# Illumina/manta

Hardware: AMD Instinct MI355X
Metric: candidate SV loci assembled+aligned per second (whole node) (higher is better)
Workload: dtype int32

## Files before the change

### manta_amd/csrc/api_internal.hpp

```cpp
#pragma once
#include "../../include/manta_amd.h"

#include <algorithm>
#include <atomic>
#include <functional>
#include <condition_variable>
#include <chrono>
#include <cstdio>
#include <cstdlib>
#include <cstring>
#include <memory>
#include <mutex>
#include <optional>
#include <string>
#include <thread>
#include <vector>

#include "align_kernels.hpp"
#include "align_jump_pair.hpp"
#include "assemble_kernels.hpp"
#include "asm_lds.hpp"
#include "small_asm.hpp"
#include "pipeline_kernels.hpp"
#include "split_kernels.hpp"
// ... 866 lines not shown
    P.bits_cap       = devBitsCap;
    P.bits_used      = reinterpret_cast<unsigned long long*>(dCnt + 2);
    P.phase_cycles   = reinterpret_cast<unsigned long long*>(dCnt + 4);
    P.growth_size    = dGrowth;
    P.growth_buckets = dGrowth + ctx->growthSize.size();
    P.n_growth       = uint32_t(ctx->growthSize.size());
    P.flags          = std::getenv("MANTA_AMD_SERIAL_WALK") ? ASM_FLAG_SERIAL_WALK : 0u;
    P.locus_min_wl   = dMinWl;
    P.locus_max_wl   = dMaxWl;
    P.locus_ids      = dOrder;
    P.pl_codes       = dPlCodes;
    P.pl_nmask       = dPlMask;
    P.pl_read_len    = dPlLen;
    P.pl_code_off    = dPlCodeOff;
    P.pl_mask_off    = dPlMaskOff;
    chunks.fill(P);
    P.reserved2          = 0;
    P.small_min_seed_reads = smallMinSeedReads;
    P.small_max_iterations = smallMaxIterations;
    P.punt_ids             = nullptr;
    P.punt_count           = nullptr;
    P.n_loci_dev           = nullptr;
    P.lds_bytes            = ASM_LDS_BYTES;
    P.stop_before          = 0;
    lastParams             = P;
    nRerun                 = 0;
    if (smallMode) {
      rt::launch(small_assemble_kernel, grid, 0, P);
      return;
    }
    int g = grid;
    if (chunks.active() && g >= ctx->cuCount * 16) g = rt::roundGrid(g - ctx->cuCount);
    P.lds_bytes = ASM_LDS_BYTES;
    if (useFast) {
      using namespace manta_dev;
      const uint32_t nGen = uint32_t(genIds.size());
      rt::h2d(reinterpret_cast<uint32_t*>(dCnt + 14), &nGen, sizeof(uint32_t));
      uint64_t* dLg = bLgCnt.as<uint64_t>(16);
      rt::dzero(dLg, sizeof(uint64_t) * 16);
      LgArgs A;
      A.P            = P;
      A.P.n_loci     = uint32_t(fastIds.size());
      A.P.punt_ids   = dPunt;
      A.P.punt_count = reinterpret_cast<uint32_t*>(dCnt + 14);
      A.G.arena        = bLgArena.as<uint8_t>(lgArenaCap + 64);
      A.G.arena_cap    = lgArenaCap;
      A.G.arena_used   = reinterpret_cast<unsigned long long*>(dLg);
      A.G.slab_off     = bLgOff.as<uint64_t>(nLoci);
      A.G.class_ids    = bLgClassIds.as<uint32_t>(uint64_t(LG_CLASSES) * std::max<size_t>(1, fastIds.size()));
      A.G.class_count  = reinterpret_cast<uint32_t*>(dLg + 1);
      A.G.class_stride = uint32_t(fastIds.size());
      for (unsigned c = 0; c < LG_CLASSES; ++c) A.G.class_bytes[c] = classBytes[c];
      A.G.cls        = 0;
      A.G.flags      = (std::getenv("MANTA_AMD_LG_NO_PROOF") ? LG_FLAG_NO_PROOF : 0u) | (std::getenv("MANTA_AMD_LG_NO_RESCUE") ? LG_FLAG_NO_RESCUE : 0u);
      A.G.stats      = reinterpret_cast<uint32_t*>(dLg + 8);
      int maxGrid = 1;
      for (unsigned c = 0; c < LG_CLASSES; ++c) maxGrid = std::max(maxGrid, gridContig[c]);
      A.G.cws        = bCws.as<uint8_t>(cwsStride * uint64_t(maxGrid));
      A.G.cws_stride = cwsStride;
      A.G.cost_bins = nullptr;
      if (contigPool && !fastIds.empty()) {
        A.G.cost_bins = bLgBins.as<uint32_t>(CK_BIN_IDS + uint64_t(CK_BINS) * fastIds.size());
        rt::dzero(A.G.cost_bins, sizeof(uint32_t) * CK_BIN_IDS);
      }
      A.G.round = A.G.last_round = 0;
      A.G.iter        = nullptr;
      A.G.parena      = nullptr;
      A.G.parena_cap  = 0;
      A.G.parena_used = nullptr;
      A.G.next_ids = A.G.next_count = A.G.cyc_ids = A.G.cyc_count = nullptr;
      A.G.rws        = nullptr;
      A.G.rws_stride = 0;
      A.G.gws        = nullptr;
      A.G.rprof      = nullptr;
      A.G.sched      = sched;
      int gf = gridFast;
      if (chunks.active() && gf >= ctx->cuCount * 2) gf -= ChunkStream::streamFreeSlots(ctx->cuCount);
      if (!fastIds.empty()) {
        uint32_t firstWl = opt.min_word_length;
        if (!locusMinWl.empty()) {
          firstWl = 0;
          for (const uint32_t l : fastIds) firstWl = std::max(firstWl, locusMinWl[l]);
        }
        if (firstWl <= 32)
          rt::launchWG(graph_kernel<2>, gf, int(LG_WAVES), LG_BUDGET, A);
        else if (firstWl <= 64)
          rt::launchWG(graph_kernel<4>, gf, int(LG_WAVES), LG_BUDGET, A);
        else
          rt::launchWG(graph_kernel<8>, gf, int(LG_WAVES), LG_BUDGET, A);
      }
      bool smallContigsLaunched = false;
      auto launchSmallContigs   = [&] {
        if (smallContigsLaunched) return;
        smallContigsLaunched = true;
        if (sched && schedWaits) rt::curStreamWaits(*schedWaits);
        for (unsigned c = 0; c < LG_CLASSES && !fastIds.empty(); ++c) {
          if (!classBytes[c]) continue;
          A.G.cls       = c;
          A.P.counter   = reinterpret_cast<uint32_t*>(dLg + 3) + c;
          A.P.lds_bytes = classBytes[c];
          if (c == 0 && contigPool)
            rt::launchWG(contig_pool_kernel, gridContig[c] / int(CK_POOL_WAVES), int(CK_POOL_WAVES), CK_POOL_BYTES, A);
          else
            rt::launchSingle(contig_kernel, gridContig[c], classBytes[c], A);
        }
      };
      firstRoundHookRan = false;
// ... 237 lines not shown
    seqCopied  = std::min<uint64_t>(cnt[1], devSeqCap);
    bitsCopied = std::min<uint64_t>(cnt[2], devBitsCap);
    hSeq       = pSeq.as<uint8_t>(seqCopied + 1);
    hBits      = pBits.as<uint64_t>(bitsCopied + 1);
    rt::d2hAsync(hCnt, dCnt, sizeof(uint64_t) * 16);
    rt::d2hAsync(hLoci, dLoci, sizeof(AsmLocusOut) * nLoci);
    rt::d2hAsync(hCont, dCont, sizeof(AsmContigOut) * uint64_t(nLoci) * opt.max_assembly_count);
    rt::d2hAsync(hSeq, dSeq, seqCopied);
    rt::d2hAsync(hBits, dBits, sizeof(uint64_t) * bitsCopied);
    done.record();
    earlyStaged = true;
  }
  void finishEarly()
  {
    seqUsedDev  = seqCopied;
    bitsUsedDev = bitsCopied;
    seqLast     = seqUsedDev;
    bitsLast    = bitsUsedDev;
    stagedTotals();
  }
  template <typename F0>
  void stageEnqueueRest(F0 firstCopies)
  {
    firstCopies();
    stageQueued = true;
  }
  void stagedTotals()
  {
    nContigsOut = pseudoBytesOut = pseudoCountOut = 0;
    for (uint32_t l = 0; l < nLoci; ++l) {
      const AsmLocusOut& h(hLoci[l]);
      if (h.status != ASM_OK) continue;
      nContigsOut += h.n_contigs;
      pseudoCountOut += h.n_pseudo;
      for (uint32_t q = 0; q < h.n_pseudo; ++q) pseudoBytesOut += hBits[h.pseudo_len_off + q];
    }
    staged = true;
    ldsFallbacks = useFast ? uint32_t(hCnt[14] & 0xffffffffu) - uint32_t(genIds.size()) : 0u;
    if (std::getenv("MANTA_AMD_DEBUG") && useFast) {
      uint32_t st[2] = {0, 0}, stBig[10] = {0, 0, 0, 0, 0, 0, 0, 0, 0, 0}, clsBig[2] = {0, 0};
      rt::d2h(st, bLgCnt.as<uint64_t>(16) + 8, sizeof(st));
      rt::d2h(stBig, bLgCnt.as<uint64_t>(16) + 11, sizeof(stBig));
      rt::d2h(clsBig, bLgCnt.as<uint64_t>(16) + 5, sizeof(clsBig));
      std::fprintf(stderr, "manta_amd: LDS assembler pipeline: %zu + %zu (big class) loci, %u handed to the general kernel (+ %zu outside its envelope); %u + %u graphs came "
                           "with a proof of acyclicity, %u + %u reads re-anchored; big class: %u / %u loci in its two contig LDS classes\n", fastIds.size(), bigIds.size(),
                   ldsFallbacks, genIds.size(), st[0], stBig[0], st[1], stBig[1], clsBig[0], clsBig[1]);
      if (contigPool && !fastIds.empty()) {
        uint32_t bins[manta_dev::CK_BIN_IDS];
        rt::d2h(bins, bLgBins.as<uint32_t>(manta_dev::CK_BIN_IDS + uint64_t(manta_dev::CK_BINS) * fastIds.size()), sizeof(bins));
        const uint32_t* ps = bins + manta_dev::CK_BIN_STAT;
        std::fprintf(stderr, "manta_amd: contig_pool_kernel: %u shares taken, %.2f loci resident per CU on average at a take, %u takes waited for room (%u polls); "
                             "loci by cost bin (largest first):", ps[0], ps[0] ? double(ps[1]) / ps[0] : 0.0, ps[2], ps[3]);
        for (unsigned b = 0; b < manta_dev::CK_BINS; ++b) std::fprintf(stderr, " %u", bins[b]);
        std::fprintf(stderr, "\n");
      }
      if (!bigIds.empty())
        std::fprintf(stderr, "manta_amd: big class, %u word-length rounds; handed back: %u envelope, %u table / set pool, %u words / side tables / class, %u slab arena, %u by "
                             "repeat_big_kernel, %u by contig_big_kernel, %u pseudo arena, %u out of rounds\n", bigRounds, stBig[2], stBig[3], stBig[4], stBig[5], stBig[6],
                     stBig[7], stBig[8], stBig[9]);
      if (bigRounds) {
        unsigned long long rp[8] = {0, 0, 0, 0, 0, 0, 0, 0}, tot = 0;
        uint32_t           perRound[8 * manta_dev::LGL_MAX_ROUNDS];
        uint32_t*          rc = bLgRounds.as<uint32_t>(8 * (manta_dev::LGL_MAX_ROUNDS + 1) + 32);
        rt::d2h(rp, rc + 8 * (manta_dev::LGL_MAX_ROUNDS + 1), sizeof(rp));
        rt::d2h(perRound, rc, sizeof(perRound));
        for (int i = 0; i < 7; ++i) tot += rp[i];
        std::fprintf(stderr, "manta_amd: repeat_big_kernel clocks: renumbering %.1f%% component scan %.1f%% hash+insertion %.1f%% order1 %.1f%% order2 %.1f%% search in the reference's order %.1f%% rest %.1f%% (%.0f k clocks per graph without a proof, first three rounds)\n",
                     tot ? 100.0 * rp[0] / tot : 0, tot ? 100.0 * rp[1] / tot : 0, tot ? 100.0 * rp[2] / tot : 0, tot ? 100.0 * rp[3] / tot : 0, tot ? 100.0 * rp[4] / tot : 0,
                     tot ? 100.0 * rp[5] / tot : 0, tot ? 100.0 * rp[6] / tot : 0, perRound[5] ? double(tot) / 1e3 / double(std::max<uint32_t>(1, perRound[5] + perRound[8 + 5] + perRound[16 + 5])) : 0.0);
        std::fprintf(stderr, "manta_amd: rounds (graphs without a proof / loci sent on):");
        for (uint32_t r = 0; r < bigRounds; ++r) std::fprintf(stderr, " %u/%u", perRound[8 * r + 5], perRound[8 * r + 7]);
        std::fprintf(stderr, "\n");
      }
    }
    if (std::getenv("MANTA_AMD_PROFILE")) {
      static const char* namesGeneral[8] = {"pack", "table", "links", "cycle-check", "exact", "seed", "walk", "select+emit"};
#ifdef MANTA_LG_PROFILE_GRAPH
      static const char* namesLds[8]     = {"pack", "table", "links", "counts+radix", "ties+ids", "slab+sets+init", "preds+sibs", "spec+write"};
#else
      static const char* namesLds[8]     = {"pack", "table", "sort+records", "cycle-check", "slab write/read", "seed+replay", "walk", "select+emit"};
#endif
      const char* const* names = useFast ? namesLds : namesGeneral;
      uint64_t           tot = 0;
      for (int i = 0; i < 8; ++i) tot += hCnt[4 + i];
      std::fprintf(stderr, "manta_amd %s phase share (shader clocks summed over %u loci; graph_kernel: clocks of one wave of the workgroup):", useFast ? "graph_kernel + contig_kernel" : "assemble_kernel", nLoci);
      for (int i = 0; i < 8; ++i) std::fprintf(stderr, " %s=%.1f%%", names[i], tot ? 100.0 * double(hCnt[4 + i]) / double(tot) : 0.0);
      std::fprintf(stderr, " | avg clocks/locus=%.0f\n", double(tot) / nLoci);
    }
  }
  void stageOut()
  {
    stageEnqueue([] {});
    rt::sync();
    stageFinish([](bool&) {});
  }

  struct SparseContigs {
    const AsmStage* st;
    const AsmContigOut& operator()(uint32_t l, uint32_t c) const { return st->hCont[uint64_t(l) * st->opt.max_assembly_count + c]; }
  };
  void exactSizes(uint64_t& nContigs, uint64_t& seqBytes, uint64_t& bitsWords) const { exactSizes(SparseContigs{this}, nContigs, seqBytes, bitsWords); }
  template <typename ContigAt>
  void exactSizes(ContigAt contigAt, uint64_t& nContigs, uint64_t& seqBytes, uint64_t& bitsWords) const
  {
    nContigs = nContigsOut;
    seqBytes = pseudoBytesOut;
    bitsWords = pseudoCountOut;
// ... 797 lines not shown
```

### manta_amd/csrc/asm_contig.hpp

```cpp
#pragma once
#ifdef MANTA_WAVE_EMU
#include <set>
#endif
#include "asm_lds.hpp"

namespace manta_dev {

#ifndef MANTA_CK_FAST_CAP
#define MANTA_CK_FAST_CAP 3
#endif
static const unsigned CK_FAST_CAP = MANTA_CK_FAST_CAP;
static const unsigned CK_MAX_EXT = 1020;

struct CkWsLayout {
  uint64_t lane_seq, lane_bits, lane_meta, lane_log, total;
};
static const unsigned CK_SEQ_WORDS = CK_MAX_EXT / 16 + 2;
static const unsigned CK_LOG_QW    = (CK_MAX_EXT + 4) / 4;
WV_HD CkWsLayout ckWorkspaceLayout(const unsigned setw = 2)
{
  CkWsLayout L;
  uint64_t   o = 0;
  L.lane_seq  = asmPut(o, 64ull * 2 * 4 * CK_SEQ_WORDS);
  L.lane_bits = asmPut(o, 64ull * 2 * setw * 8);
  L.lane_meta = asmPut(o, 64ull * 8 * 4);
  L.lane_log  = asmPut(o, 64ull * 8 * CK_LOG_QW);
  L.total     = (o + 255) & ~uint64_t(255);
  return L;
}

enum { CK_DONE = 0, CK_PUNT = 1, CK_NEXT = 2 };

template <class C>
struct LdsContig {
  typedef LgRec<C>  R;
  typedef FSetT<C>  Set;
  typedef CkMap<C>  M;
  static const unsigned SW  = C::SETW;
  static const unsigned IDB = C::ID_BITS;
  static const unsigned IDM = (1u << C::ID_BITS) - 1u;
  static const unsigned UPL = C::UNUSED_DW / 64;
  const AsmParams& P;
  const LgParams&  G;
  char*            lds;
  const uint8_t*   slab;
  FRec8*           nodes;
  Set*             pool;
  uint8_t*         rd1;
  uint32_t*        unused_bits;
  uint16_t *       tent, *slotNode, *sib, *sovf, *povf;
  LgSlab           SL;
  uint8_t*         tbl;
  uint32_t*        lane_seq;
  uint64_t*        lane_bits;
  int32_t*         lane_meta;
  uint64_t*        lane_log;
  unsigned         lane, nNormal, W, k, nNodes, nFat, nEligible, nSpec, nSib, nSovf, nPovf, codeWords, nCand, maxLen, seqWords;
  bool             acyclic;
  bool             cyclic, anyRep;
  unsigned         nPseudo, nCore, visDw;
  uint32_t *       coreBits, *repBits, *vis;
  uint16_t*        corePrefix;
  unsigned         candSlotV;
  uint64_t         tMark;
  unsigned         shareBytes;

  WV_DEV LdsContig(const AsmParams& p, const LgParams& g, char* base, uint8_t* ws) : P(p), G(g), lds(base)
  {
    lane        = unsigned(wv::lane());
    unused_bits = reinterpret_cast<uint32_t*>(lds + M::UNUSED);
    tent        = reinterpret_cast<uint16_t*>(lds + M::TENT);
    slotNode    = reinterpret_cast<uint16_t*>(lds + M::SLOTND);
    tbl         = reinterpret_cast<uint8_t*>(lds + M::TBL);
    sib         = reinterpret_cast<uint16_t*>(lds + M::SIB);
    sovf        = reinterpret_cast<uint16_t*>(lds + M::SOVF);
    povf        = reinterpret_cast<uint16_t*>(lds + M::POVF);
    nodes       = reinterpret_cast<FRec8*>(lds + M::RECS);
    pool        = nullptr;
    rd1         = nullptr;
    const CkWsLayout L = ckWorkspaceLayout(SW);
    lane_seq  = reinterpret_cast<uint32_t*>(ws + L.lane_seq);
    lane_bits = reinterpret_cast<uint64_t*>(ws + L.lane_bits);
    lane_meta = reinterpret_cast<int32_t*>(ws + L.lane_meta);
    lane_log  = reinterpret_cast<uint64_t*>(ws + L.lane_log);
    maxLen    = p.max_contig_len;
    seqWords  = CK_SEQ_WORDS;
    candSlotV = 0;
    nCand     = 0;
    shareBytes = 0;
    cyclic = anyRep = false;
    nPseudo = nCore = visDw = 0;
    coreBits = repBits = vis = nullptr;
    corePrefix = nullptr;
  }

  WV_DEV void tick(const int phase)
  {
#if defined(MANTA_ASM_PROFILE) && !defined(MANTA_LG_PROFILE_GRAPH)
    const uint64_t now = wv::clock();
    if (P.phase_cycles && lane == 0) wv::atomic_add(&P.phase_cycles[phase], (unsigned long long)(now - tMark));
    tMark = now;
#else
    (void)phase;
#endif
  }

  WV_DEV bool isUnused(const unsigned nd) const { return (unused_bits[nd >> 5] >> (nd & 31)) & 1u; }
  WV_DEV char*    scratch() const { return lds + M::RECS + ((8 * nNodes + 15) & ~15u) + (C::BIG ? ((nNodes + 15) & ~15u) : 0u); }

  WV_DEV unsigned onlyRead(const unsigned nd, const FRec8 w) const { return C::BIG ? unsigned(rd1[nd]) : lg8Read(w); }
  WV_DEV Set supOf(const unsigned nd, const FRec8 w) const
  {
    Set s;
    if (nd < nFat) {
      s = pool[nd];
    } else {
      const unsigned ref = onlyRead(nd, w);
      for (unsigned q = 0; q < SW; ++q) s.w[q] = ((ref >> 6) == q) ? (uint64_t(1) << (ref & 63)) : 0;
    }
    return s;
  }
  WV_DEV uint64_t succOf(const unsigned nd, const FRec8 w) const { return R::links(w, nd, true, sovf, nSovf); }
  WV_DEV uint64_t predOf(const unsigned nd, const FRec8 w) const { return R::links(w, nd, false, povf, nPovf); }
  WV_DEV static unsigned popSet(const Set& a)
  {
    unsigned n = 0;
    for (unsigned q = 0; q < SW; ++q) n += unsigned(wv::popc(a.w[q]));
    return n;
  }
  WV_DEV static Set setAnd(const Set& a, const Set& b)
  {
    Set r;
    for (unsigned q = 0; q < SW; ++q) r.w[q] = a.w[q] & b.w[q];
    return r;
  }
  WV_DEV static Set setAndNot(const Set& a, const Set& b)
  {
    Set r;
    for (unsigned q = 0; q < SW; ++q) r.w[q] = a.w[q] & ~b.w[q];
    return r;
  }
  WV_DEV static void setOrIn(Set& a, const Set& b)
  {
    for (unsigned q = 0; q < SW; ++q) a.w[q] |= b.w[q];
  }
  WV_DEV static Set setZero()
  {
    Set r;
    for (unsigned q = 0; q < SW; ++q) r.w[q] = 0;
    return r;
  }
  WV_DEV static Set setSel(const bool c, const Set& a, const Set& b)
  {
    Set r;
    for (unsigned q = 0; q < SW; ++q) r.w[q] = c ? a.w[q] : b.w[q];
    return r;
  }

  WV_DEV bool load(const unsigned locus)
  {
    slab            = G.arena + G.slab_off[locus];
    const LgHdr* gh = reinterpret_cast<const LgHdr*>(slab);
    nNodes          = wv::first(gh->nNodes);
    nFat            = wv::first(gh->nFat);
    k               = wv::first(gh->k);
    nNormal         = wv::first(gh->nNormal);
    nEligible       = wv::first(gh->nEligible);
    nSpec           = wv::first(gh->nSpec);
    nSib            = wv::first(gh->nSib);
    nSovf           = wv::first(gh->nSovf);
    nPovf           = wv::first(gh->nPovf);
    codeWords       = wv::first(gh->codeWords);
    W               = wv::first(gh->W);
    acyclic         = wv::first(gh->acyclic) != 0;
    cyclic          = C::BIG && wv::first(gh->cyclic) != 0;
    nPseudo         = C::BIG ? wv::first(gh->nPseudo) : 0u;
    nCore           = cyclic ? wv::first(gh->nCore) : 0u;
    if (wv::first(gh->need) > P.lds_bytes || nNodes > C::MAX_NODES) return false;
    SL               = lgSlabOf<C>(nNodes, nFat, codeWords);
    const FRec8* gRec = reinterpret_cast<const FRec8*>(slab + SL.recs);
    for (unsigned i = lane; i < nNodes; i += 64) nodes[i] = gRec[i];
    if (C::BIG) {
      rd1                 = reinterpret_cast<uint8_t*>(lds + M::RECS + ((8 * nNodes + 15) & ~15u));
      const uint32_t* g4  = reinterpret_cast<const uint32_t*>(slab + SL.rd1);
      uint32_t*       l4  = reinterpret_cast<uint32_t*>(rd1);
      for (unsigned i = lane; i < (nNodes + 3) / 4; i += 64) l4[i] = g4[i];
    }
    const uint16_t* gt = reinterpret_cast<const uint16_t*>(slab + SL.sib);
    for (unsigned i = lane; i < 4 * (LG_SIB_CAP + 2 * C::OVF_CAP); i += 64) sib[i] = gt[i];
    for (unsigned u = 0; u < UPL; ++u) {
      const unsigned d = UPL * lane + u, lo = 32 * d;
      unused_bits[d]   = (nEligible >= lo + 32) ? 0xffffffffu : ((nEligible > lo) ? ((1u << (nEligible - lo)) - 1u) : 0u);
    }
    if (cyclic) {
      char* x    = scratch() + 8 * SW * (nFat ? nFat : 1u);
      coreBits   = reinterpret_cast<uint32_t*>(x);
      corePrefix = reinterpret_cast<uint16_t*>(x + 4 * C::UNUSED_DW);
      repBits    = reinterpret_cast<uint32_t*>(x + 6 * C::UNUSED_DW);
      vis        = reinterpret_cast<uint32_t*>(x + 10 * C::UNUSED_DW);
      visDw      = (nCore + 31) / 32;
      const uint32_t* gf = reinterpret_cast<const uint32_t*>(slab + SL.flags);
      unsigned        c  = 0;
      uint32_t        cb[UPL];
      for (unsigned u = 0; u < UPL; ++u) {
        const unsigned d = UPL * lane + u;
        cb[u]            = gf[d];
        coreBits[d]      = cb[u];
        repBits[d]       = gf[C::UNUSED_DW + d];
        c += unsigned(wv::popc(cb[u]));
      }
      unsigned inc = c;
      for (int off = 1; off < 64; off <<= 1) {
        const unsigned o = wv::shfl(inc, int(lane) - off);
        if (int(lane) >= off) inc += o;
      }
      unsigned at = inc - c;
      for (unsigned u = 0; u < UPL; ++u) {
        corePrefix[UPL * lane + u] = uint16_t(at);
        at += unsigned(wv::popc(cb[u]));
      }
      wv::sync();
      for (unsigned u = 0; u < UPL; ++u) {
        uint32_t b32 = cb[u];
        while (b32) {
          const unsigned b = unsigned(wv::ctz(uint64_t(b32)));
          b32 &= b32 - 1;
          nodes[32 * (UPL * lane + u) + b] |= FRec8(1) << 63;
        }
      }
    }
    wv::sync();
    return true;
  }
  WV_DEV static bool coreFlag(const FRec8 w) { return C::BIG && (w >> 63) != 0; }
  WV_DEV unsigned    coreIndex(const unsigned nd) const
  {
    return unsigned(corePrefix[nd >> 5]) + unsigned(wv::popc(coreBits[nd >> 5] & ((1u << (nd & 31)) - 1u)));
  }
  WV_DEV const Set*      gPool() const { return reinterpret_cast<const Set*>(slab + SL.pool); }
  WV_DEV const uint16_t* gSpecList() const { return reinterpret_cast<const uint16_t*>(slab + SL.spec); }
  WV_DEV const uint16_t* gPb() const { return reinterpret_cast<const uint16_t*>(slab + SL.pb); }
  WV_DEV const uint32_t* gCodes() const { return reinterpret_cast<const uint32_t*>(slab + SL.codes); }

  WV_DEV void loadPool()
  {
    pool              = reinterpret_cast<Set*>(scratch());
    const Set* gp     = gPool();
    for (unsigned i = lane; i < nFat; i += 64) pool[i] = gp[i];
    if (nFat == 0 && lane == 0) pool[0] = setZero();
    wv::sync();
  }

  WV_DEV bool graphHasCycle()
  {
    const unsigned stDw = (nNodes + 3) / 4;
    uint32_t*      st    = reinterpret_cast<uint32_t*>(scratch());
    uint32_t*      qTail = st + stDw;
    uint16_t*      queue = reinterpret_cast<uint16_t*>(qTail + 4);
    if (lane == 0) *qTail = 0;
    for (unsigned w = lane; w < stDw; w += 64) st[w] = 0;
    wv::sync();
    for (unsigned nb = 0; nb < nNodes; nb += 64) {
      const unsigned nd = nb + lane;
      if (nd >= nNodes) continue;
      const FRec8    w  = nodes[nd];
      const uint64_t sl = succOf(nd, w), pl = predOf(nd, w);
      unsigned       id = 0, od = 0;
      for (unsigned c = 0; c < 4; ++c) {
        const unsigned s = R::linkId(sl, c), p = R::linkId(pl, c);
        if (s != ASM_NONE && s != nd) od++;
        if (p != ASM_NONE && p != nd) id++;
      }
      const bool     src = (id == 0 || od == 0);
      const unsigned v   = id | (od << 3) | (src ? 0x40u : 0u);
      wv::atomic_or(&st[nd >> 2], v << (8 * (nd & 3)));
      if (src) queue[wv::atomic_add(qTail, 1u)] = uint16_t(nd);
    }
    wv::sync();
    unsigned head = 0, removed = 0;
    while (true) {
      const unsigned tail = wv::first(wv::atomic_load(qTail));
      if (tail == head) break;
      removed += tail - head;
      for (unsigned i = head + lane; i < tail; i += 64) {
        const unsigned nd = queue[i];
        const FRec8    w  = nodes[nd];
        const uint64_t sl = succOf(nd, w), pl = predOf(nd, w);
        for (unsigned c = 0; c < 4; ++c) {
          const unsigned s = R::linkId(sl, c);
          if (s != ASM_NONE && s != nd) {
            const unsigned sh  = 8 * (s & 3);
            const unsigned old = wv::atomic_sub(&st[s >> 2], 1u << sh) >> sh;
            if ((old & 0x7u) == 1u && !(wv::atomic_or(&st[s >> 2], 0x40u << sh) & (0x40u << sh))) queue[wv::atomic_add(qTail, 1u)] = uint16_t(s);
          }
          const unsigned p = R::linkId(pl, c);
          if (p != ASM_NONE && p != nd) {
            const unsigned sh  = 8 * (p & 3);
            const unsigned old = wv::atomic_sub(&st[p >> 2], 8u << sh) >> sh;
            if ((old & 0x38u) == 8u && !(wv::atomic_or(&st[p >> 2], 0x40u << sh) & (0x40u << sh))) queue[wv::atomic_add(qTail, 1u)] = uint16_t(p);
          }
        }
      }
// ... 64 lines not shown
    unsigned ent[WIN], lab[WIN];
    for (unsigned h = 0; h < WIN; ++h) {
      const unsigned i = lane + 64 * h;
      ent[h]           = (i < nW) ? unsigned(tent[i]) : ASM_NONE;
      unsigned cur     = (i < nW) ? ent[h] : 0u;
      for (unsigned steps = 0; steps < 256 && i < nW; ++steps) {
        const FRec8    w  = nodes[cur];
        const unsigned f0 = R::succ(w, 0);
        if (f0 == 0 || R::succ(w, 1) != 0 || R::sOvf(w) || f0 - 1 == cur) break;
        const FRec8 wn = nodes[f0 - 1];
        if (R::pred(wn, 1) != 0 || R::pOvf(wn)) break;
        cur = f0 - 1;
      }
      lab[h] = (i < nW) ? cur : (ASM_NONE - 1u - i);
    }
    bool dup[WIN];
    for (unsigned h = 0; h < WIN; ++h) dup[h] = false;
    for (unsigned g = 0; g < WIN; ++g) {
      const unsigned gEnd = (nW > 64 * g) ? ((nW - 64 * g < 64) ? (nW - 64 * g) : 64u) : 0u;
      for (unsigned j = 0; j < gEnd; ++j) {
        const unsigned v = wv::readlane(lab[g], int(j));
        for (unsigned h = g; h < WIN; ++h)
          if (64 * g + j < lane + 64 * h && v == lab[h] && lane + 64 * h >= PLAIN) dup[h] = true;
      }
    }
    unsigned base = 0;
    uint64_t keepM[WIN];
    for (unsigned h = 0; h < WIN; ++h) keepM[h] = wv::ballot(ent[h] != ASM_NONE && !dup[h]);
#ifdef MANTA_WAVE_EMU
    if (emuWhy()) {
      for (unsigned h = 0; h < WIN; ++h)
        if (ent[h] != ASM_NONE) {
          dbg().looked.insert(ent[h]);
          if (dup[h]) dbg().dropped.insert(ent[h]);
        }
    }
#endif
    const uint64_t below = (uint64_t(1) << lane) - 1;
    wv::sync();
    for (unsigned h = 0; h < WIN; ++h) {
      if ((keepM[h] >> lane) & 1u) tent[base + unsigned(wv::popc(keepM[h] & below))] = uint16_t(ent[h]);
      base += unsigned(wv::popc(keepM[h]));
    }
    wv::sync();
    return (base < 64) ? base : 64u;
  }

  struct Cand {
    FRec8 w;
    Set   s;
  };

  WV_DEV FRec8    candRec(const unsigned f) const { return nodes[f ? f - 1 : 0]; }
  WV_DEV Set      candPool(const unsigned f) const { return pool[(f != 0 && f - 1 < nFat) ? f - 1 : 0u]; }
  WV_DEV unsigned candRd1(const unsigned f) const { return C::BIG ? unsigned(rd1[f ? f - 1 : 0]) : 0u; }
  WV_DEV Set      candSup(const unsigned f, const FRec8 w, const Set& p, const unsigned r1) const
  {
    const unsigned ref  = C::BIG ? r1 : lg8Read(w);
    const bool     fat  = f != 0 && f - 1 < nFat;
    const uint64_t useM = fat ? ~uint64_t(0) : 0;
    const uint64_t bit  = uint64_t((f != 0 && !fat) ? 1u : 0u) << (ref & 63);
    Set            s;
    if (SW == 2) {
      const uint64_t hiM = (ref & 64u) ? ~uint64_t(0) : 0;
      s.w[0]             = (p.w[0] & useM) | (bit & ~hiM);
      s.w[1]             = (p.w[1] & useM) | (bit & hiM);
    } else {
      for (unsigned q = 0; q < SW; ++q) s.w[q] = (p.w[q] & useM) | (((ref >> 6) == q) ? bit : 0);
    }
    return s;
  }
  WV_DEV Cand loadCand(const unsigned f) const
  {
    Cand           c;
    const Set      p  = candPool(f);
    const unsigned r1 = candRd1(f);
    c.w               = candRec(f);
    c.s               = candSup(f, c.w, p, r1);
    return c;
  }

  WV_DEV void walkSlots(const uint64_t walkMask)
  {
    const bool has = (walkMask >> lane) & 1u;
    LG_STAT(1, 1);
    LG_STAT(2, unsigned(wv::popc(walkMask)));
    const unsigned seed = has ? unsigned(slotNode[lane]) : 0u;
    uint64_t* const logBuf   = lane_log + lane;
    uint64_t        logAcc   = seed;
    uint32_t* const rightBuf = lane_seq + lane;
    uint32_t* const leftBuf  = lane_seq + 64 + lane;
    uint32_t       accR = 0, accL = 0;
    Set            S = setZero(), RJ = setZero();
    bool           active = has, rep = false, tooLong = false;
    unsigned       mode = 0, cur = seed, consOffset = 0, nLeft = 0, nRight = 0;
    int            consEnd = 0, consBegin = 0;
    FRec8          seedRec = 0;
    if (cyclic && has)
      for (unsigned w = 0; w < visDw; ++w) vis[w * 64 + lane] = 0;
    if (has) {
      seedRec = nodes[seed];
      S       = supOf(seed, seedRec);
      const bool repeatSeed = R::selfLoop(seedRec) || (cyclic && ((repBits[seed >> 5] >> (seed & 31)) & 1u));
      if (repeatSeed) {
        rep    = true;
        active = false;
      } else {
// ... 856 lines not shown
    wv::sync();
    if (rc == CK_PUNT && wv::lane() == 0) P.punt_ids[wv::atomic_add(P.punt_count, 1u)] = locus;
    wv::sync();
  }
}
#if !MANTA_TU_DEFINES(MANTA_TU_CONTIG)
WV_KERNEL_SINGLE WV_WAVES_PER_SIMD(2) void contig_kernel(const LgArgs A);
#else
WV_KERNEL_SINGLE WV_WAVES_PER_SIMD(2) void contig_kernel(const LgArgs A)
{
  contigKernelBody<LgS>(A);
}
#endif

static const unsigned CK_POOL_WAVES = 12;
static const unsigned CK_POOL_BYTES = 163840;
static const unsigned CK_POOL_HDR   = 64;
static_assert(4 * (1 + CK_POOL_WAVES) <= CK_POOL_HDR && (CK_POOL_BYTES - CK_POOL_HDR) / 16 < 65536, "pool header");

WV_DEV unsigned ckPoolTake(char* pool, const unsigned w, const unsigned units, uint32_t* stat)
{
  uint32_t*      lock  = reinterpret_cast<uint32_t*>(pool);
  uint32_t*      share = lock + 1;
  const unsigned lane  = unsigned(wv::lane());
  const unsigned capU  = (CK_POOL_BYTES - CK_POOL_HDR) / 16;
  unsigned       polls = 0;
  while (true) {
    ++polls;
    unsigned got = 0;
    if (lane == 0) got = (wv::atomic_cas(lock, 0u, 1u) == 0u) ? 1u : 0u;
    if (wv::first(got)) {
      wv::fence_wg();
      unsigned s = 0;
      if (lane >= 1 && lane <= CK_POOL_WAVES) s = wv::atomic_load(&share[lane - 1]) >> 16;
      bool ok = lane <= CK_POOL_WAVES && s + units <= capU;
      for (unsigned v = 0; v < CK_POOL_WAVES; ++v) {
        const unsigned e = wv::atomic_load(&share[v]), a = e & 0xffffu, b = e >> 16;
        if (a < b && s < b && a < s + units) ok = false;
      }
      const uint64_t m  = wv::ballot(ok);
      const unsigned at = m ? wv::readlane(s, wv::ctz(m)) : 0u;
      if (m && lane == 0) wv::atomic_store(&share[w], at | ((at + units) << 16));
      const unsigned e        = (lane < CK_POOL_WAVES) ? wv::atomic_load(&share[lane]) : 0u;
      const bool     held     = (e & 0xffffu) < (e >> 16);
      const unsigned resident = unsigned(wv::popc(wv::ballot(held)));
      wv::fence_wg();
      if (lane == 0) wv::atomic_exch(lock, 0u);
      if (m) {
        if (stat && lane == 0) {
          wv::atomic_add(&stat[0], 1u);
          wv::atomic_add(&stat[1], resident);
          if (polls > 1) wv::atomic_add(&stat[2], 1u);
          wv::atomic_add(&stat[3], polls);
        }
        return CK_POOL_HDR + 16 * at;
      }
    }
    wv::sleep();
  }
}

template <class C>
WV_DEV void contigPoolBody(const LgArgs& A)
{
  const AsmParams& P    = A.P;
  const LgParams&  G    = A.G;
  const unsigned   w    = unsigned(wv::wave_in_wg());
  uint8_t*         ws   = G.cws + (uint64_t(wv::block_single()) * unsigned(wv::wg_waves()) + w) * G.cws_stride;
  char*            pool = wv::lds_single();
  if (w == 0 && wv::lane() <= int(CK_POOL_WAVES)) reinterpret_cast<uint32_t*>(pool)[wv::lane()] = 0u;
  wv::wg_barrier();
  const unsigned  nLoci = wv::first(wv::atomic_load(&G.class_count[G.cls]));
  const uint32_t* ids   = G.class_ids + size_t(G.cls) * G.class_stride;
  const unsigned  capU  = (P.lds_bytes + 15) / 16;
  const unsigned lane   = unsigned(wv::lane());
  unsigned       binLen = 0, binAt = 0;
  if (G.cost_bins) {
    binLen = (lane < CK_BINS) ? wv::atomic_load(&G.cost_bins[lane]) : 0u;
    binAt  = binLen;
    for (int off = 1; off < 64; off <<= 1) {
      const unsigned o = wv::shfl(binAt, int(lane) - off);
      if (int(lane) >= off) binAt += o;
    }
    binAt -= binLen;
  }
  while (true) {
    unsigned slot = 0;
    if (lane == 0) slot = wv::atomic_add(P.counter, 1u);
    slot = wv::first(slot);
    if (slot >= nLoci) break;
    unsigned locus;
    if (G.cost_bins) {
      const uint64_t inBin = wv::ballot(lane < CK_BINS && slot >= binAt && slot < binAt + binLen);
      const unsigned b     = unsigned(wv::ctz(inBin));
      locus                = G.cost_bins[CK_BIN_IDS + size_t(b) * G.class_stride + (slot - wv::readlane(binAt, int(b)))];
    } else {
      locus = ids[slot];
    }
    const LgHdr*   gh    = reinterpret_cast<const LgHdr*>(G.arena + G.slab_off[locus]);
    const unsigned needU = (wv::first(gh->need) + 15) / 16;
    const unsigned units = (needU < capU) ? needU : capU;
    char*          lds   = pool + ckPoolTake(pool, w, units, G.cost_bins ? G.cost_bins + CK_BIN_STAT : nullptr);
    LdsContig<C>   c(P, G, lds, ws);
    c.shareBytes = 16 * units;
    const int      rc = c.run(locus);
    wv::sync();
    if (wv::lane() == 0) wv::atomic_store(reinterpret_cast<uint32_t*>(pool) + 1 + w, 0u);
    if (rc == CK_PUNT && wv::lane() == 0) P.punt_ids[wv::atomic_add(P.punt_count, 1u)] = locus;
    wv::sync();
  }
}
#if !MANTA_TU_DEFINES(MANTA_TU_CONTIG)
WV_KERNEL_WG(CK_POOL_WAVES) WV_WAVES_PER_SIMD(3) void contig_pool_kernel(const LgArgs A);
#else
WV_KERNEL_WG(CK_POOL_WAVES) WV_WAVES_PER_SIMD(3) void contig_pool_kernel(const LgArgs A)
{
  contigPoolBody<LgS>(A);
}
#endif
#if !MANTA_TU_DEFINES(MANTA_TU_CONTIG)
WV_KERNEL_SINGLE WV_WAVES_PER_SIMD(1) void contig_big_kernel(const LgArgs A);
#else
WV_KERNEL_SINGLE WV_WAVES_PER_SIMD(1) void contig_big_kernel(const LgArgs A)
{
  contigKernelBody<LgL>(A);
}
#endif

}

#include "asm_lds_big.hpp"
#include "asm_repeat_big.hpp"
```

### manta_amd/csrc/asm_lds.hpp

```cpp
#pragma once
#include "assemble_kernels.hpp"
#include "smallsv_trim.hpp"

namespace manta_dev {

static const unsigned LG_SLOTS     = 2048;
static const unsigned LG_BUCKETS   = LG_SLOTS / 4;
static const unsigned LG_MAX_NODES = 1843;
static const unsigned LG_MAX_READS = 128;
static const unsigned LG_MAX_PILE  = 2046;
static const unsigned LG_EMPTY     = 0xffffffffu;
static const unsigned LG_FAT       = 0x800u;
static const unsigned LG_NO_SLOT   = 0xffffu;
static const unsigned LG_WAVES     = 8;
static const unsigned LG_BUDGET    = 81920;
static const unsigned LG_SIB_CAP   = 32;
static const unsigned LG_OVF_CAP   = 32;
static const unsigned LG_CLASSES   = 4;
static const unsigned CK_BINS     = 8;
static const unsigned CK_BIN_STAT = CK_BINS;
static const unsigned CK_BIN_IDS  = 16;

static const unsigned LG_OFF_HDR   = 0;
static const unsigned LG_OFF_RD    = 512;
// ... 58 lines not shown
};
WV_HD LgSlab lgSlab(const unsigned nNodes, const unsigned nFat, const unsigned codeWords)
{
  LgSlab   L;
  uint32_t o = uint32_t(sizeof(LgHdr));
  L.rd1   = 0;
  L.lex   = 0;
  L.flags = 0;
  L.recs  = o;
  o += (8u * nNodes + 15u) & ~15u;
  L.pool  = o;
  o += 16u * nFat;
  L.spec  = o;
  o += 128u;
  L.sib   = o;
  o += 8u * LG_SIB_CAP;
  L.sovf  = o;
  o += 8u * LG_OVF_CAP;
  L.povf  = o;
  o += 8u * LG_OVF_CAP;
  L.pb    = o;
  o += (2u * nNodes + 15u) & ~15u;
  L.codes = o;
  o += (4u * codeWords + 15u) & ~15u;
  L.total = o;
  return L;
}
WV_HD uint64_t lgSlabBytes(const unsigned nNodes, const unsigned nFat, const unsigned codeWords)
{
  return lgSlab(nNodes, nFat, codeWords).total;
}
WV_HD bool lgPileFits(const uint64_t nReads, const uint64_t maxAssemblyCount, const uint64_t cw, const uint64_t mw, const uint64_t longest)
{
  if (nReads + 2 * maxAssemblyCount > LG_MAX_READS) return false;
  if (longest > 0xffffu || cw + 2 > LG_MAX_PILE) return false;
  const uint64_t cwPad = (cw + 2 + 3) & ~uint64_t(3), mwPad = (mw + 2 + 3) & ~uint64_t(3);
  return LG_OFF_DYN + 4 * (cwPad + mwPad) <= LG_BUDGET;
}

static const unsigned CK_OFF_HDR    = 0;
static const unsigned CK_OFF_UNUSED = 64;
static const unsigned CK_OFF_TENT   = 320;
static const unsigned CK_OFF_SLOTND = 576;
static const unsigned CK_OFF_TBL    = 704;
static const unsigned CK_OFF_SIB    = 768;
static const unsigned CK_OFF_SOVF   = CK_OFF_SIB + 8 * LG_SIB_CAP;
static const unsigned CK_OFF_POVF   = CK_OFF_SOVF + 8 * LG_OVF_CAP;
static const unsigned CK_OFF_RECS   = CK_OFF_POVF + 8 * LG_OVF_CAP;
WV_HD unsigned ckNeed(const unsigned nNodes, const unsigned nFat, const bool acyclic)
{
  const unsigned kahn = acyclic ? 0u : ((4 * ((nNodes + 3) / 4) + 2 * nNodes + 32 + 15) & ~15u);
  const unsigned pool = 16 * (nFat ? nFat : 1u);
  return CK_OFF_RECS + ((8 * nNodes + 15) & ~15u) + ((pool > kahn) ? pool : kahn);
}

static const unsigned LGL_SLOTS     = 8192;
static const unsigned LGL_BUCKETS   = LGL_SLOTS / 4;
static const unsigned LGL_MAX_NODES = 7168;
static const unsigned LGL_MAX_READS = 256;
static const unsigned LGL_MAX_PILE  = 3598;
static const unsigned LGL_MAX_PILE_ALL = 4090;
static const unsigned LGL_POOL_CAP  = 1280;
static const unsigned LGL_POOL_OVF  = 704;
static const unsigned LGL_GWS_SETS  = 32 * LGL_POOL_OVF;
static const unsigned LGL_GWS_BYTES = LGL_GWS_SETS + 2 * 8192 + 2 * 8192;
static const unsigned LGL_WAVES     = 16;
static const unsigned LGL_BUDGET    = 163840;
static const unsigned LGL_OVF_CAP   = 128;
static const unsigned LGL_CLASSES   = 2;

struct LgS {
  static const bool     BIG       = false;
  static const unsigned ID_BITS   = 11;
  static const unsigned SETW      = 2;
  static const unsigned MAX_NODES = LG_MAX_NODES;
  static const unsigned OVF_CAP   = LG_OVF_CAP;
  static const unsigned UNUSED_DW = 64;
  static const unsigned CNT_SH = 44, FIRST_SH = 55, LAST_SH = 57, SELF_SH = 59, SOVF_SH = 60, POVF_SH = 61;
};
WV_DEV unsigned lg8Read(const FRec8 w) { return unsigned(w >> 48) & 0x7fu; }
struct LgL {
  static const bool     BIG       = true;
  static const unsigned ID_BITS   = 13;
  static const unsigned SETW      = 4;
  static const unsigned MAX_NODES = LGL_MAX_NODES;
  static const unsigned OVF_CAP   = LGL_OVF_CAP;
  static const unsigned UNUSED_DW = 256;
  static const unsigned CNT_SH = 52, FIRST_SH = 56, LAST_SH = 58, SELF_SH = 60, SOVF_SH = 61, POVF_SH = 62;
};
template <class C>
struct alignas(16) FSetT {
  uint64_t w[C::SETW];
};
template <class C>
struct LgRec {
  static const unsigned IDM  = (1u << C::ID_BITS) - 1u;
  static const uint64_t M2   = (uint64_t(1) << (2 * C::ID_BITS)) - 1;
  WV_DEV static unsigned succ(const FRec8 w, const unsigned i) { return unsigned(w >> (C::ID_BITS * i)) & IDM; }
  WV_DEV static unsigned pred(const FRec8 w, const unsigned i) { return unsigned(w >> (C::ID_BITS * (2 + i))) & IDM; }
  WV_DEV static unsigned cnt(const FRec8 w) { return unsigned(w >> C::CNT_SH) & 15u; }
  WV_DEV static unsigned firstBase(const FRec8 w) { return unsigned(w >> C::FIRST_SH) & 3u; }
  WV_DEV static unsigned lastBase(const FRec8 w) { return unsigned(w >> C::LAST_SH) & 3u; }
  WV_DEV static bool     selfLoop(const FRec8 w) { return (w >> C::SELF_SH) & 1u; }
  WV_DEV static bool     sOvf(const FRec8 w) { return (w >> C::SOVF_SH) & 1u; }
  WV_DEV static bool     pOvf(const FRec8 w) { return (w >> C::POVF_SH) & 1u; }
  WV_DEV static uint64_t links(const FRec8 w, const unsigned nd, const bool succ, const uint16_t* ovf, const unsigned nOvf)
// ... 26 lines not shown
  o += (8u * nNodes + 15u) & ~15u;
  L.pool  = o;
  o += 32u * nFat;
  L.spec  = o;
  o += 128u;
  L.sib   = o;
  o += 8u * LG_SIB_CAP;
  L.sovf  = o;
  o += 8u * LGL_OVF_CAP;
  L.povf  = o;
  o += 8u * LGL_OVF_CAP;
  L.rd1   = o;
  o += (nNodes + 15u) & ~15u;
  L.pb    = o;
  o += (2u * nNodes + 15u) & ~15u;
  L.codes = o;
  o += (4u * codeWords + 15u) & ~15u;
  L.lex   = o;
  o += (2u * nNodes + 15u) & ~15u;
  L.flags = o;
  o += 8u * 256u;
  L.total = o;
  return L;
}
template <class C>
WV_HD LgSlab lgSlabOf(const unsigned nNodes, const unsigned nFat, const unsigned codeWords)
{
  return C::BIG ? lgSlabL(nNodes, nFat, codeWords) : lgSlab(nNodes, nFat, codeWords);
}

#ifndef MANTA_STRETCH_WIN
#define MANTA_STRETCH_WIN 4
#endif
static const unsigned LGL_STRETCH_WIN = MANTA_STRETCH_WIN;
template <class C>
struct CkMap {
  static const unsigned UNUSED = 64;
  static const unsigned TENT   = UNUSED + 4 * C::UNUSED_DW;
  static const unsigned SLOTND = TENT + (C::BIG ? 2 * 64 * LGL_STRETCH_WIN : 256);
  static const unsigned TBL    = SLOTND + 128;
  static const unsigned SIB    = TBL + 64;
  static const unsigned SOVF   = SIB + 8 * LG_SIB_CAP;
  static const unsigned POVF   = SOVF + 8 * C::OVF_CAP;
  static const unsigned RECS   = POVF + 8 * C::OVF_CAP;
};
static_assert(CkMap<LgS>::TENT == CK_OFF_TENT && CkMap<LgS>::SLOTND == CK_OFF_SLOTND && CkMap<LgS>::TBL == CK_OFF_TBL && CkMap<LgS>::SIB == CK_OFF_SIB &&
              CkMap<LgS>::RECS == CK_OFF_RECS, "the small class keeps its map");
template <class C>
WV_HD unsigned ckNeedOf(const unsigned nNodes, const unsigned nFat, const bool acyclic)
{
  const unsigned kahn = acyclic ? 0u : ((4 * ((nNodes + 3) / 4) + 2 * nNodes + 32 + 15) & ~15u);
  const unsigned pool = 8 * C::SETW * (nFat ? nFat : 1u);
  return CkMap<C>::RECS + ((8 * nNodes + 15) & ~15u) + (C::BIG ? ((nNodes + 15) & ~15u) : 0u) + ((pool > kahn) ? pool : kahn);
}

static const unsigned LGL_CORE_CAP = 4096;
template <class C>
WV_HD unsigned ckCyclicExtra(const unsigned nCore)
{
  return 4u * C::UNUSED_DW + 2u * C::UNUSED_DW + 4u * C::UNUSED_DW + 64u * 4u * ((nCore + 31u) / 32u);
}
template <class C>
WV_HD unsigned ckNeedCyclic(const unsigned nNodes, const unsigned nFat, const unsigned nCore)
{
  const unsigned pool = 8 * C::SETW * (nFat ? nFat : 1u);
  return CkMap<C>::RECS + ((8 * nNodes + 15) & ~15u) + (C::BIG ? ((nNodes + 15) & ~15u) : 0u) + pool + ckCyclicExtra<C>(nCore);
}

static const unsigned LGL_MAX_PSEUDO = 40;
static const unsigned LGL_MAX_ROUNDS = 24;
struct alignas(16) LgIter {
  uint32_t k;
  uint32_t nIter;
  uint32_t cyclicIters;
  uint32_t nPseudo;
  uint64_t off;
  uint32_t codeWords;
  uint32_t slabCap;
  uint16_t len[LGL_MAX_PSEUDO];
};

struct LgParams;
struct LgArgs;
struct LgParams {
  uint8_t*            arena;
  uint64_t            arena_cap;
  unsigned long long* arena_used;
  uint64_t*           slab_off;
  uint32_t*           class_ids;
  uint32_t*           class_count;
  uint32_t            class_stride;
  uint32_t            class_bytes[LG_CLASSES];
  uint32_t            cls;
  uint32_t            flags;
  uint32_t*           stats;
  uint8_t*            cws;
  uint32_t*           cost_bins;
  uint64_t            cws_stride;
  uint32_t            round;
  uint32_t            last_round;
  LgIter*             iter;
  uint32_t*           parena;
  uint64_t            parena_cap;
  unsigned long long* parena_used;
  uint32_t*           next_ids;
  uint32_t*           next_count;
  uint32_t*           cyc_ids;
  uint32_t*           cyc_count;
  uint8_t*            rws;
  uint64_t            rws_stride;
  uint8_t*            gws;
  unsigned long long* rprof;
  const ScheduleParams* sched;
};

static const uint32_t LG_FLAG_NO_PROOF = 1u;
static const uint32_t LG_FLAG_NO_RESCUE = 2u;

struct LgArgs {
  AsmParams P;
  LgParams  G;
};

#ifdef MANTA_WAVE_EMU
inline unsigned long long* fastStats()
{
  static unsigned long long v[8] = {0, 0, 0, 0, 0, 0, 0, 0};
  return v;
}
#define LG_STAT(i, n) do { if (wv::lane() == 0) fastStats()[i] += (n); } while (0)
#else
#define LG_STAT(i, n) do { } while (0)
#endif

}

#include "asm_lds_base.hpp"

namespace manta_dev {

struct LdsGraph : LdsGraphBase<LgGraphS> {
  typedef LgRec<LgS> R;
  uint32_t *       slots, *keyArr;
  uint16_t *       sortA, *sortB, *slotId;
  uint8_t*         cntArr;
  FSet*            sets;
  FRec8*           nodes;
  uint64_t*        pred4;
  int16_t*         phi;
  int16_t*         roff;
  uint32_t*        filter;

  WV_DEV LdsGraph(const AsmParams& p, const LgParams& g, char* base) : LdsGraphBase<LgGraphS>(p, g, base)
  {
    slots  = reinterpret_cast<uint32_t*>(lds + LG_OFF_SLOTS);
    sets   = reinterpret_cast<FSet*>(lds + LG_OFF_SETS);
    nodes  = reinterpret_cast<FRec8*>(lds + LG_OFF_SETS);
    pred4  = reinterpret_cast<uint64_t*>(lds + LG_OFF_SETS) + LG_SLOTS;
    phi    = reinterpret_cast<int16_t*>(lds + LG_OFF_PHI);
    roff   = reinterpret_cast<int16_t*>(lds + LG_OFF_RDM);
    filter = reinterpret_cast<uint32_t*>(lds + LG_OFF_FILTER);
    sortA  = reinterpret_cast<uint16_t*>(lds + LG_OFF_SORTA);
    sortB  = reinterpret_cast<uint16_t*>(lds + LG_OFF_SORTB);
    keyArr = reinterpret_cast<uint32_t*>(lds + LG_OFF_KEYS);
    slotId = reinterpret_cast<uint16_t*>(lds + LG_OFF_KEYS);
    cntArr = reinterpret_cast<uint8_t*>(lds + LG_OFF_CNT);
  }

  template <int KW>
  WV_DEV unsigned lookupSlot(const Key<KW>& key) const
// ... 667 lines not shown
```

Baseline: 1.325 million.

## Size small-class LDS shares to actual sibling/overflow counts and pack sets to 12 bytes

For the small class, the per-locus LDS layout now sizes the sibling and overflow tables from the locus's actual counts instead of fixed caps, and stores fat-node read sets with a 12-byte stride when the read count allows it. The pool scheduler takes shares sized from this compact layout, so more loci should fit in each CU's LDS pool at once. The cost is extra index arithmetic on every set load, a new layout path that must match the slab contents, and a new env flag that restores the wide layout. A debug statistic reporting the mean share size is also added.

```diff
diff --git a/manta_amd/csrc/api_internal.hpp b/manta_amd/csrc/api_internal.hpp
--- a/manta_amd/csrc/api_internal.hpp
+++ b/manta_amd/csrc/api_internal.hpp
@@ -942,7 +942,8 @@
       A.G.class_stride = uint32_t(fastIds.size());
       for (unsigned c = 0; c < LG_CLASSES; ++c) A.G.class_bytes[c] = classBytes[c];
       A.G.cls        = 0;
-      A.G.flags      = (std::getenv("MANTA_AMD_LG_NO_PROOF") ? LG_FLAG_NO_PROOF : 0u) | (std::getenv("MANTA_AMD_LG_NO_RESCUE") ? LG_FLAG_NO_RESCUE : 0u);
+      A.G.flags      = (std::getenv("MANTA_AMD_LG_NO_PROOF") ? LG_FLAG_NO_PROOF : 0u) | (std::getenv("MANTA_AMD_LG_NO_RESCUE") ? LG_FLAG_NO_RESCUE : 0u) |
+                       (std::getenv("MANTA_AMD_WIDE_SHARES") ? LG_FLAG_WIDE_SHARES : 0u);
       A.G.stats      = reinterpret_cast<uint32_t*>(dLg + 8);
       int maxGrid = 1;
       for (unsigned c = 0; c < LG_CLASSES; ++c) maxGrid = std::max(maxGrid, gridContig[c]);
@@ -1286,7 +1287,7 @@
         std::fprintf(stderr, "manta_amd: contig_pool_kernel: %u shares taken, %.2f loci resident per CU on average at a take, %u takes waited for room (%u polls); "
                              "loci by cost bin (largest first):", ps[0], ps[0] ? double(ps[1]) / ps[0] : 0.0, ps[2], ps[3]);
         for (unsigned b = 0; b < manta_dev::CK_BINS; ++b) std::fprintf(stderr, " %u", bins[b]);
-        std::fprintf(stderr, "\n");
+        std::fprintf(stderr, "; mean share %.0f bytes\n", ps[0] ? 16.0 * double(ps[4]) / ps[0] : 0.0);
       }
       if (!bigIds.empty())
         std::fprintf(stderr, "manta_amd: big class, %u word-length rounds; handed back: %u envelope, %u table / set pool, %u words / side tables / class, %u slab arena, %u by "
diff --git a/manta_amd/csrc/asm_contig.hpp b/manta_amd/csrc/asm_contig.hpp
--- a/manta_amd/csrc/asm_contig.hpp
+++ b/manta_amd/csrc/asm_contig.hpp
@@ -46,6 +46,8 @@
   const uint8_t*   slab;
   FRec8*           nodes;
   Set*             pool;
+  char*            scr;
+  bool             set12;
   uint8_t*         rd1;
   uint32_t*        unused_bits;
   uint16_t *       tent, *slotNode, *sib, *sovf, *povf;
@@ -73,11 +75,12 @@
     slotNode    = reinterpret_cast<uint16_t*>(lds + M::SLOTND);
     tbl         = reinterpret_cast<uint8_t*>(lds + M::TBL);
     sib         = reinterpret_cast<uint16_t*>(lds + M::SIB);
-    sovf        = reinterpret_cast<uint16_t*>(lds + M::SOVF);
-    povf        = reinterpret_cast<uint16_t*>(lds + M::POVF);
-    nodes       = reinterpret_cast<FRec8*>(lds + M::RECS);
+    sovf = povf = nullptr;
+    nodes       = nullptr;
     pool        = nullptr;
     rd1         = nullptr;
+    scr         = nullptr;
+    set12       = false;
     const CkWsLayout L = ckWorkspaceLayout(SW);
     lane_seq  = reinterpret_cast<uint32_t*>(ws + L.lane_seq);
     lane_bits = reinterpret_cast<uint64_t*>(ws + L.lane_bits);
@@ -106,14 +109,23 @@
   }
 
   WV_DEV bool isUnused(const unsigned nd) const { return (unused_bits[nd >> 5] >> (nd & 31)) & 1u; }
-  WV_DEV char*    scratch() const { return lds + M::RECS + ((8 * nNodes + 15) & ~15u) + (C::BIG ? ((nNodes + 15) & ~15u) : 0u); }
+  WV_DEV char*    scratch() const { return scr; }
+  WV_DEV Set poolAt(const unsigned i) const
+  {
+    if (C::BIG) return pool[i];
+    Set             s;
+    const uint32_t* d = reinterpret_cast<const uint32_t*>(scr + (set12 ? 12u : 16u) * i);
+    s.w[0]            = uint64_t(d[0]) | (uint64_t(d[1]) << 32);
+    s.w[1]            = uint64_t(d[2]) | (uint64_t(set12 ? 0u : d[3]) << 32);
+    return s;
+  }
 
   WV_DEV unsigned onlyRead(const unsigned nd, const FRec8 w) const { return C::BIG ? unsigned(rd1[nd]) : lg8Read(w); }
   WV_DEV Set supOf(const unsigned nd, const FRec8 w) const
   {
     Set s;
     if (nd < nFat) {
-      s = pool[nd];
+      s = poolAt(nd);
     } else {
       const unsigned ref = onlyRead(nd, w);
       for (unsigned q = 0; q < SW; ++q) s.w[q] = ((ref >> 6) == q) ? (uint64_t(1) << (ref & 63)) : 0;
@@ -178,16 +190,30 @@
     nCore           = cyclic ? wv::first(gh->nCore) : 0u;
     if (wv::first(gh->need) > P.lds_bytes || nNodes > C::MAX_NODES) return false;
     SL               = lgSlabOf<C>(nNodes, nFat, codeWords);
+    const CkLayout LY = ckLayoutOf<C>(nNodes, nFat, nSib, nSovf, nPovf, nNormal, acyclic, (G.flags & LG_FLAG_WIDE_SHARES) != 0);
+    sovf             = reinterpret_cast<uint16_t*>(lds + LY.sovf);
+    povf             = reinterpret_cast<uint16_t*>(lds + LY.povf);
+    nodes            = reinterpret_cast<FRec8*>(lds + LY.recs);
+    scr              = lds + LY.sets;
+    set12            = LY.set12;
     const FRec8* gRec = reinterpret_cast<const FRec8*>(slab + SL.recs);
     for (unsigned i = lane; i < nNodes; i += 64) nodes[i] = gRec[i];
     if (C::BIG) {
-      rd1                 = reinterpret_cast<uint8_t*>(lds + M::RECS + ((8 * nNodes + 15) & ~15u));
+      rd1                 = reinterpret_cast<uint8_t*>(lds + LY.rd1);
       const uint32_t* g4  = reinterpret_cast<const uint32_t*>(slab + SL.rd1);
       uint32_t*       l4  = reinterpret_cast<uint32_t*>(rd1);
       for (unsigned i = lane; i < (nNodes + 3) / 4; i += 64) l4[i] = g4[i];
     }
-    const uint16_t* gt = reinterpret_cast<const uint16_t*>(slab + SL.sib);
-    for (unsigned i = lane; i < 4 * (LG_SIB_CAP + 2 * C::OVF_CAP); i += 64) sib[i] = gt[i];
+    if (C::BIG) {
+      const uint16_t* gt = reinterpret_cast<const uint16_t*>(slab + SL.sib);
+      for (unsigned i = lane; i < 4 * (LG_SIB_CAP + 2 * C::OVF_CAP); i += 64) sib[i] = gt[i];
+    } else {
+      const uint16_t *gs = reinterpret_cast<const uint16_t*>(slab + SL.sib), *go = reinterpret_cast<const uint16_t*>(slab + SL.sovf),
+                     *gp = reinterpret_cast<const uint16_t*>(slab + SL.povf);
+      for (unsigned i = lane; i < 4 * nSib; i += 64) sib[i] = gs[i];
+      for (unsigned i = lane; i < 4 * nSovf; i += 64) sovf[i] = go[i];
+      for (unsigned i = lane; i < 4 * nPovf; i += 64) povf[i] = gp[i];
+    }
     for (unsigned u = 0; u < UPL; ++u) {
       const unsigned d = UPL * lane + u, lo = 32 * d;
       unused_bits[d]   = (nEligible >= lo + 32) ? 0xffffffffu : ((nEligible > lo) ? ((1u << (nEligible - lo)) - 1u) : 0u);
@@ -244,10 +270,22 @@
 
   WV_DEV void loadPool()
   {
-    pool              = reinterpret_cast<Set*>(scratch());
     const Set* gp     = gPool();
-    for (unsigned i = lane; i < nFat; i += 64) pool[i] = gp[i];
-    if (nFat == 0 && lane == 0) pool[0] = setZero();
+    if (C::BIG) {
+      pool = reinterpret_cast<Set*>(scratch());
+      for (unsigned i = lane; i < nFat; i += 64) pool[i] = gp[i];
+      if (nFat == 0 && lane == 0) pool[0] = setZero();
+    } else {
+      const unsigned nSet = nFat ? nFat : 1u, stride = set12 ? 12u : 16u;
+      for (unsigned i = lane; i < nSet; i += 64) {
+        const Set s = (i < nFat) ? gp[i] : setZero();
+        uint32_t* d = reinterpret_cast<uint32_t*>(scr + stride * i);
+        d[0]        = uint32_t(s.w[0]);
+        d[1]        = uint32_t(s.w[0] >> 32);
+        d[2]        = uint32_t(s.w[1]);
+        if (!set12) d[3] = uint32_t(s.w[1] >> 32);
+      }
+    }
     wv::sync();
   }
 
@@ -418,7 +456,7 @@
   };
 
   WV_DEV FRec8    candRec(const unsigned f) const { return nodes[f ? f - 1 : 0]; }
-  WV_DEV Set      candPool(const unsigned f) const { return pool[(f != 0 && f - 1 < nFat) ? f - 1 : 0u]; }
+  WV_DEV Set      candPool(const unsigned f) const { return poolAt((f != 0 && f - 1 < nFat) ? f - 1 : 0u); }
   WV_DEV unsigned candRd1(const unsigned f) const { return C::BIG ? unsigned(rd1[f ? f - 1 : 0]) : 0u; }
   WV_DEV Set      candSup(const unsigned f, const FRec8 w, const Set& p, const unsigned r1) const
   {
@@ -1381,6 +1419,7 @@
           wv::atomic_add(&stat[1], resident);
           if (polls > 1) wv::atomic_add(&stat[2], 1u);
           wv::atomic_add(&stat[3], polls);
+          wv::atomic_add(&stat[4], units);
         }
         return CK_POOL_HDR + 16 * at;
       }
@@ -1427,7 +1466,18 @@
       locus = ids[slot];
     }
     const LgHdr*   gh    = reinterpret_cast<const LgHdr*>(G.arena + G.slab_off[locus]);
-    const unsigned needU = (wv::first(gh->need) + 15) / 16;
+    const unsigned need  = wv::first(gh->need);
+    unsigned       share = ckLayoutOf<C>(wv::first(gh->nNodes), wv::first(gh->nFat), wv::first(gh->nSib), wv::first(gh->nSovf), wv::first(gh->nPovf),
+                                         wv::first(gh->nNormal), wv::first(gh->acyclic) != 0, (G.flags & LG_FLAG_WIDE_SHARES) != 0).total;
+    if (G.sched) {
+      const ScheduleParams& S   = *G.sched;
+      const uint64_t        ro0 = wv::readlane(uint64_t(S.ref_off[locus]), 0), ro1 = wv::readlane(uint64_t(S.ref_off[locus + 1]), 0);
+      const uint64_t        ref = (ro1 >= ro0) ? ro1 - ro0 : 0;
+      const unsigned        sch = (ref < need) ? SCHED_TABLE_BYTES + schedStagedBytes(512, unsigned(ref)) : need;
+      const unsigned        cap = (sch < need) ? sch : need;
+      if (share < cap) share = cap;
+    }
+    const unsigned needU = (share + 15) / 16;
     const unsigned units = (needU < capU) ? needU : capU;
     char*          lds   = pool + ckPoolTake(pool, w, units, G.cost_bins ? G.cost_bins + CK_BIN_STAT : nullptr);
     LdsContig<C>   c(P, G, lds, ws);
diff --git a/manta_amd/csrc/asm_lds.hpp b/manta_amd/csrc/asm_lds.hpp
--- a/manta_amd/csrc/asm_lds.hpp
+++ b/manta_amd/csrc/asm_lds.hpp
@@ -134,6 +134,33 @@
   const unsigned kahn = acyclic ? 0u : ((4 * ((nNodes + 3) / 4) + 2 * nNodes + 32 + 15) & ~15u);
   const unsigned pool = 16 * (nFat ? nFat : 1u);
   return CK_OFF_RECS + ((8 * nNodes + 15) & ~15u) + ((pool > kahn) ? pool : kahn);
+}
+struct CkLayout {
+  uint32_t unused, tent, slotnd, tbl, sib, sovf, povf, recs, rd1, sets, total;
+  uint32_t setStride;
+  bool     set12;
+};
+WV_HD CkLayout ckShare(const unsigned nNodes, const unsigned nFat, const unsigned nSib, const unsigned nSovf, const unsigned nPovf, const unsigned nNormal,
+                       const bool acyclic, const bool wide)
+{
+  CkLayout       L;
+  const unsigned kahn = acyclic ? 0u : ((4 * ((nNodes + 3) / 4) + 2 * nNodes + 32 + 15) & ~15u);
+  const unsigned nSet = nFat ? nFat : 1u;
+  L.set12       = !wide && nNormal <= 96;
+  L.unused      = CK_OFF_UNUSED;
+  L.tent        = CK_OFF_TENT;
+  L.slotnd      = CK_OFF_SLOTND;
+  L.tbl         = CK_OFF_TBL;
+  L.sib         = CK_OFF_SIB;
+  L.sovf        = L.sib + ((8 * (wide ? LG_SIB_CAP : nSib) + 15) & ~15u);
+  L.povf        = L.sovf + ((8 * (wide ? LG_OVF_CAP : nSovf) + 15) & ~15u);
+  L.recs        = L.povf + ((8 * (wide ? LG_OVF_CAP : nPovf) + 15) & ~15u);
+  L.rd1         = 0;
+  L.sets        = L.recs + ((8 * nNodes + 15) & ~15u);
+  L.setStride   = L.set12 ? 12u : 16u;
+  const unsigned pool = L.set12 ? ((12 * nSet + 15) & ~15u) : 16 * nSet;
+  L.total       = L.sets + ((pool > kahn) ? pool : kahn);
+  return L;
 }
 
 static const unsigned LGL_SLOTS     = 8192;
@@ -266,6 +293,28 @@
   const unsigned kahn = acyclic ? 0u : ((4 * ((nNodes + 3) / 4) + 2 * nNodes + 32 + 15) & ~15u);
   const unsigned pool = 8 * C::SETW * (nFat ? nFat : 1u);
   return CkMap<C>::RECS + ((8 * nNodes + 15) & ~15u) + (C::BIG ? ((nNodes + 15) & ~15u) : 0u) + ((pool > kahn) ? pool : kahn);
+}
+
+template <class C>
+WV_HD CkLayout ckLayoutOf(const unsigned nNodes, const unsigned nFat, const unsigned nSib, const unsigned nSovf, const unsigned nPovf, const unsigned nNormal,
+                          const bool acyclic, const bool wide)
+{
+  if (!C::BIG) return ckShare(nNodes, nFat, nSib, nSovf, nPovf, nNormal, acyclic, wide);
+  CkLayout L;
+  L.set12       = false;
+  L.unused      = CkMap<C>::UNUSED;
+  L.tent        = CkMap<C>::TENT;
+  L.slotnd      = CkMap<C>::SLOTND;
+  L.tbl         = CkMap<C>::TBL;
+  L.sib         = CkMap<C>::SIB;
+  L.sovf        = CkMap<C>::SOVF;
+  L.povf        = CkMap<C>::POVF;
+  L.recs        = CkMap<C>::RECS;
+  L.rd1         = L.recs + ((8 * nNodes + 15) & ~15u);
+  L.sets        = L.rd1 + ((nNodes + 15) & ~15u);
+  L.setStride   = 8 * C::SETW;
+  L.total       = ckNeedOf<C>(nNodes, nFat, acyclic);
+  return L;
 }
 
 static const unsigned LGL_CORE_CAP = 4096;
@@ -330,6 +379,7 @@
 
 static const uint32_t LG_FLAG_NO_PROOF = 1u;
 static const uint32_t LG_FLAG_NO_RESCUE = 2u;
+static const uint32_t LG_FLAG_WIDE_SHARES = 4u;
 
 struct LgArgs {
   AsmParams P;
```

Result: slower. 1.311 million (-1.1%).
